# kwea123/nsff_pl

Hardware: AMD Instinct MI355X
Metric: ray-samples/sec (coarse+fine, static+dynamic) (higher is better)
Workload: dtype f16x3 (fp32 operands split into 2 halfs, 3 f16 MFMAs per product, fp32 accumulate; same 1e-4 parity as f32); 1 GPU; C2 (BASELINE.json configs[1]): static+dynamic NSFF, 1024 rays/GPU x (64 coarse + 64 importance -> 192 fine pts), train-mode fwd, fw/bw flow warp t+-1, perturb=1 noise_std=1, 8x256 MLPs, N_tau=48, all 47 outputs on device.  `value` is render_rays' throughput with autograd DISABLED (the train-mode FLAGS, inference launches: nothing kept for a backward pass); what a trainer's forward costs is aux.tra; rays_per_gpu=1024, N_samples=64, N_importance=64, parallelism=single GPU, field_launch=persistent (one workgroup per CU)

## Files before the change

include/nsff_render.h:

```cpp
#ifndef NSFF_RENDER_H
#define NSFF_RENDER_H

#include <stddef.h>
#include <stdint.h>

#ifdef __cplusplus
extern "C" {
#endif

#define NSFF_OK               0
#define NSFF_ERR_INVALID     -1
#define NSFF_ERR_NULL        -2
#define NSFF_ERR_ALIGN       -3
#define NSFF_ERR_HIP         -4

#define NSFF_ABI_VERSION      32
#define NSFF_RAW_STRIDE      16
#define NSFF_MAX_FREQS       24
#define NSFF_MAX_LAYERS       8


typedef struct NsffModelDesc {
    int32_t D;
    int32_t W;
// ... 287 lines not shown
    float* static_sigmas; float* transient_sigmas;
    float* static_alphas; float* transient_alphas;
    float* static_weights; float* transient_weights; float* weights;
    float* xyzs_fw_bw;   float* xyzs_bw_fw;
    float* disoccs_fw;   float* disoccs_bw;
    float* depth;  float* rgb;  float* transient_alpha;  float* transient_rgb;
    float* static_only_rgb;  float* static_only_depth;
    float* xyz_exp;  float* flow_fw_exp;  float* flow_bw_exp;  float* xyz_fw_exp;  float* xyz_bw_exp;
    float* rgb_fw;   float* rgb_bw;
    float* disocc_fw;  float* disocc_bw;
    NsffFrustumArgs vis;
} NsffCompositeArgs;

int nsff_composite(const NsffCompositeArgs* args, void* stream);

int nsff_frustum_visibility(const NsffFrustumArgs* vis, const float* xyz, int64_t n_points, float* vis_count,
                            void* stream);

typedef struct NsffSplatArgs {
    int32_t H, W, n_planes;
    float   K4[4];
    float   P[12];
    float   scale;
    const float* xyz;
    const float* flow;
    const float* rgb;
    const float* alpha;
    float*       accum;
    void*        work;
    int64_t      work_bytes;
// ... 112 lines not shown
```

nsff_pl_amd/_lib.py:

```python
import ctypes as C
import os

import torch

_HERE = os.path.dirname(os.path.abspath(__file__))
LIB_PATH = os.environ.get("NSFF_LIB") or os.path.join(_HERE, "libnsff_hip.so")

RAW_STRIDE = 16
ABI_VERSION = 32
MAX_FREQS = 24

_ERR = {-1: "NSFF_ERR_INVALID (bad shape/flag/unsupported architecture)",
        -2: "NSFF_ERR_NULL (required pointer missing)",
        -3: "NSFF_ERR_ALIGN (pointer not 16-byte aligned)",
        -4: "NSFF_ERR_HIP"}

_fp = C.c_void_p


class ModelDesc(C.Structure):
    _fields_ = [("D", C.c_int32), ("W", C.c_int32), ("skip", C.c_int32),
                ("in_xyz", C.c_int32), ("in_dir", C.c_int32), ("in_a", C.c_int32),
                ("in_t", C.c_int32), ("use_viewdir", C.c_int32),
                ("has_transient", C.c_int32), ("has_flow", C.c_int32),
# ... 161 lines not shown
    "nsff_param_count": (C.c_int, [C.POINTER(ModelDesc)]),
    "nsff_pack_weights": (C.c_int, [C.POINTER(ModelDesc), C.c_int, C.POINTER(_fp), _fp, _fp]),
    "nsff_pack_weights_ex": (C.c_int, [C.POINTER(ModelDesc), C.c_int, C.POINTER(_fp), _fp, C.c_int32, _fp]),
    "nsff_fold_heads": (C.c_int, [C.POINTER(ModelDesc), C.c_int, C.POINTER(_fp), _fp, _fp]),
    "nsff_posenc": (C.c_int, [_fp, C.c_int64, C.POINTER(C.c_float), C.c_int, _fp, _fp]),
    "nsff_time_rows": (C.c_int, [_fp, C.c_int64, C.c_int32, _fp, C.c_int64, C.c_int64, _fp, _fp, _fp]),
    "nsff_time_rows_backward": (C.c_int, [_fp, _fp, _fp, _fp, C.c_int64, C.c_int64, C.c_int64, C.c_int32, _fp, _fp]),
    "nsff_field_query": (C.c_int, [C.POINTER(ModelDesc), _fp, C.POINTER(FieldArgs), _fp]),
    "nsff_coarse_samples": (C.c_int, [_fp, C.c_int64, _fp, C.c_int32, C.c_float, _fp, _fp, _fp, _fp]),
    "nsff_fine_samples": (C.c_int, [_fp, C.c_int64, _fp, _fp, C.c_int32, C.c_int32, _fp, _fp, _fp, _fp,
                                    C.c_int32, _fp, _fp, _fp, _fp, _fp]),
    "nsff_sample_pdf": (C.c_int, [_fp, _fp, C.c_int64, C.c_int32, _fp, C.c_int32, C.c_int32,
                                  C.c_float, _fp, _fp]),
    "nsff_warp_points": (C.c_int, [_fp, _fp, _fp, C.c_int64, C.c_float, _fp, _fp, _fp]),
    "nsff_composite": (C.c_int, [C.POINTER(CompositeArgs), _fp]),
    "nsff_frustum_visibility": (C.c_int, [C.POINTER(FrustumArgs), _fp, C.c_int64, _fp, _fp]),
    "nsff_frame_rays": (C.c_int, [C.POINTER(C.c_float), C.POINTER(C.c_float), C.c_int32, C.c_int32, C.c_float,
                                  C.c_float, C.c_int64, C.c_int64, _fp, _fp]),
    "nsff_bwd_packed_bytes": (C.c_int, [C.POINTER(ModelDesc), C.POINTER(C.c_size_t)]),
    "nsff_pack_weights_bwd": (C.c_int, [C.POINTER(ModelDesc), C.POINTER(_fp), _fp, _fp]),
    "nsff_field_backward": (C.c_int, [C.POINTER(ModelDesc), _fp, C.POINTER(FieldBwdArgs), _fp]),
    "nsff_field_input_backward": (C.c_int, [_fp, C.c_int32, C.c_int32, _fp, C.c_int64, C.c_int32, C.POINTER(C.c_float), C.c_int32,
                                            C.c_int32, _fp, _fp, _fp]),
    "nsff_train_dims": (C.c_int, [C.POINTER(ModelDesc), C.POINTER(C.c_int32), C.POINTER(C.c_int32), C.POINTER(C.c_int32)]),
    "nsff_weight_grad_scratch": (C.c_int64, [C.POINTER(WgradJob), C.c_int32, C.c_int64, C.c_int32]),
    "nsff_weight_grad": (C.c_int, [C.POINTER(WgradJob), C.c_int32, C.c_int64, C.c_int32, _fp, _fp, _fp, _fp, _fp]),
    "nsff_weight_grad_accumulate": (C.c_int, [C.POINTER(WgradJob), C.c_int32, C.c_int64, C.c_int32, _fp, _fp, C.c_int64,
                                              _fp, _fp, _fp]),
    "nsff_weight_grad_accumulate_aux": (C.c_int, [C.POINTER(WgradJob), C.c_int32, C.c_int64, C.c_int32, _fp, _fp, C.c_int64,
                                                  _fp, _fp, _fp, _fp]),
# ... 17 lines not shown
    "nsff_nerfw_loss_work_bytes": (C.c_size_t, [C.c_longlong]),
    "nsff_nerfw_loss_ex": (C.c_int, [C.POINTER(LossArgs), C.c_int, _fp, C.c_size_t, _fp]),
    "nsff_last_loss_path": (C.c_int, []),
    "nsff_splat_planes": (C.c_int, [C.POINTER(SplatArgs), _fp]),
    "nsff_splat_work_bytes": (C.c_int64, [C.c_int32, C.c_int32, C.c_int32]),
    "nsff_mpi_composite": (C.c_int, [C.POINTER(MpiArgs), _fp]),
    "nsff_ssim_scratch_bytes": (C.c_int64, [C.c_int32, C.c_int32, C.c_int32]),
    "nsff_ssim": (C.c_int, [C.POINTER(SsimArgs), _fp]),
    "nsff_cdf": (C.c_int, [_fp, C.c_int64, C.c_int64, _fp, _fp]),
    "nsff_ray_draw": (C.c_int, [C.POINTER(RayDrawArgs), _fp]),
    "nsff_prof_enable": (C.c_int, [C.c_int]),
    "nsff_prof_collect": (C.c_int, [C.POINTER(C.c_int64), C.POINTER(C.c_double), C.POINTER(C.c_double), C.POINTER(C.c_double)]),
    "nsff_prof_collect_clock": (C.c_int, [C.POINTER(C.c_int64)] + [C.POINTER(C.c_double)] * 5),
}
EXPORTED_SYMBOLS = tuple(_SIGNATURES)

_lib = None


def load():
    global _lib
    if _lib is None:
        if not os.path.exists(LIB_PATH):
            raise RuntimeError(
                f"{LIB_PATH} is missing: build it with `python -c 'import __graft_entry__ as g; g.build()'` "
                "(or `make -C nsff_pl_amd/csrc`).  There is no CPU fallback for the render path.")
        lib = C.CDLL(LIB_PATH)
        for name, (res, args) in _SIGNATURES.items():
            fn = getattr(lib, name)
            fn.restype, fn.argtypes = res, args
        if lib.nsff_abi_version() != ABI_VERSION:
            raise RuntimeError("libnsff_hip.so ABI version mismatch")
        _lib = lib
    return _lib


def _check(rc, what):
    if rc != 0:
        msg = _ERR.get(rc, f"error {rc}")
        if rc == -4:
            msg += ": " + load().nsff_last_hip_error().decode()
        raise RuntimeError(f"{what} failed: {msg}")

# ... 358 lines not shown

def frustum_args(w2c, ts, K4, n_cams, n_frames, H, W):
    assert w2c.is_cuda and w2c.dtype == torch.float32 and w2c.is_contiguous() and w2c.shape == (n_cams * n_frames, 12)
    assert ts.is_cuda and ts.dtype == torch.int64 and ts.is_contiguous() and ts.numel() >= 1
    a = FrustumArgs(w2c=w2c.data_ptr(), ts=ts.data_ptr(), n_cams=int(n_cams), n_frames=int(n_frames), H=int(H), W=int(W))
    a.K4[:] = [float(v) for v in K4]
    a._keep = (w2c, ts)
    return a


def frustum_visibility(vis, xyz, out):
    _check(load().nsff_frustum_visibility(C.byref(vis), _ptr(xyz), xyz.shape[0], _ptr(out), _stream()),
           "nsff_frustum_visibility")


def composite(vis=None, **kw):
    a = CompositeArgs()
    for k, v in kw.items():
        if k in _COMPOSITE_PTRS_IN or k in _COMPOSITE_PTRS_OUT:
            setattr(a, k, _ptr(v))
        else:
            setattr(a, k, v)
    if vis is not None:
        a.vis = vis
    _check(load().nsff_composite(C.byref(a), _stream()), "nsff_composite")


def frame_rays(K4, c2w12, H, W, near, shift_near, first, count, rays):
    k = (C.c_float * 4)(*[float(v) for v in K4])
    m = (C.c_float * 12)(*[float(v) for v in c2w12])
    _check(load().nsff_frame_rays(k, m, int(H), int(W), float(near), float(shift_near), int(first), int(count),
                                  _ptr(rays), _stream()), "nsff_frame_rays")


BWD_PACK = 100


def bwd_packed_bytes(desc):
    n = C.c_size_t(0)
    _check(load().nsff_bwd_packed_bytes(C.byref(desc), C.byref(n)), "nsff_bwd_packed_bytes")
# ... 324 lines not shown
```

nsff_pl_amd/csrc/rays.hip:

```cpp
#include <hip/hip_runtime.h>
#include <cstdlib>
#include "nsff_common.h"

namespace {

constexpr int WAVES_PER_BLOCK = 4;
constexpr int RS = NSFF_RAW_STRIDE;

__device__ __forceinline__ float wave_sum(float v) {
#pragma unroll
    for (int off = 32; off > 0; off >>= 1) v += __shfl_xor(v, off);
    return v;
}

__device__ __forceinline__ float wave_scan_mul(float v, int lane) {
#pragma unroll
    for (int off = 1; off < 64; off <<= 1) {
        const float u = __shfl_up(v, off);
        if (lane >= off) v *= u;
    }
    return v;
}
__device__ __forceinline__ float wave_scan_add(float v, int lane) {
#pragma unroll
// ... 60 lines not shown
            if (out_b) out_b[k] = s;
        }
    }
    __syncthreads();
}

struct FineArgs {
    const float* rays; long long n_rays; const float* z_lin; const float* zs_coarse;
    int S, n_imp;
    const float* w_static; const float* w_transient;
    const float* u_static; const float* u_transient; int u_per_ray;
    float* samples_static; float* samples_transient;
    float* zs_fine; float* xyz_fine;
};

__global__ __launch_bounds__(64 * WAVES_PER_BLOCK) void fine_samples_kernel(const FineArgs a) {
    extern __shared__ __attribute__((aligned(16))) float smem[];
    const int lane = threadIdx.x & 63, wave = threadIdx.x >> 6, tid = threadIdx.x;
    constexpr int T = 64 * WAVES_PER_BLOCK;
    const long long ray = blockIdx.x;
    const int S = a.S, n_imp = a.n_imp;
    const int k_sets = a.w_transient ? 2 : 1;
    const int Sf = S + k_sets * n_imp;
    float* cdf = smem + wave * S;
    float* bins = smem + WAVES_PER_BLOCK * S;
    float* merged = bins + ((S + 3) & ~3);
    for (int j = tid; j < S - 1; j += T) bins[j] = 0.5f * (a.z_lin[j] + a.z_lin[j + 1]);
    for (int j = tid; j < S; j += T) merged[j] = a.zs_coarse[ray * S + j];
    __syncthreads();
    {
        const bool mine = wave < k_sets;
        const int set = mine ? wave : 0;
        const float* w = (set == 0 ? a.w_static : a.w_transient) + ray * S + 1;
        const float* ub = set == 0 ? a.u_static : a.u_transient;
        const float* u = a.u_per_ray ? ub + ray * n_imp : ub;
        float* keep = set == 0 ? a.samples_static : a.samples_transient;
        sample_pdf_ray(w, bins, S - 2, 1e-5f, u, n_imp, cdf, merged + S + set * n_imp,
                       keep ? keep + ray * n_imp : nullptr, lane, mine);
    }
    const float* r = a.rays + ray * 6;
    const float o0 = r[0], o1 = r[1], o2 = r[2], d0 = r[3], d1 = r[4], d2 = r[5];
    for (int i = tid; i < Sf; i += T) {
        const float v = merged[i];
        int rank = 0;
        int j = 0;
        for (; j + 4 <= Sf; j += 4) {
            const float4 o = *reinterpret_cast<const float4*>(merged + j);
            rank += (o.x < v || (o.x == v && j < i)) ? 1 : 0;
            rank += (o.y < v || (o.y == v && j + 1 < i)) ? 1 : 0;
            rank += (o.z < v || (o.z == v && j + 2 < i)) ? 1 : 0;
            rank += (o.w < v || (o.w == v && j + 3 < i)) ? 1 : 0;
        }
        for (; j < Sf; ++j) {
            const float o = merged[j];
            rank += (o < v || (o == v && j < i)) ? 1 : 0;
        }
        const long long dst = ray * Sf + rank;
        a.zs_fine[dst] = v;
        a.xyz_fine[dst * 3 + 0] = o0 + d0 * v;
        a.xyz_fine[dst * 3 + 1] = o1 + d1 * v;
        a.xyz_fine[dst * 3 + 2] = o2 + d2 * v;
    }
}

struct PdfArgs {
    const float* bins; const float* weights; long long n_rays; int M;
    const float* u; int n_imp; int u_per_ray; float eps; float* samples;
};

__global__ __launch_bounds__(64 * WAVES_PER_BLOCK) void sample_pdf_kernel(const PdfArgs a) {
    extern __shared__ __attribute__((aligned(16))) float smem[];
    const int lane = threadIdx.x & 63, wave = threadIdx.x >> 6;
    const long long ray_raw = (long long)blockIdx.x * WAVES_PER_BLOCK + wave;
    const bool active = ray_raw < a.n_rays;
    const long long ray = active ? ray_raw : a.n_rays - 1;
    float* cdf = smem + wave * (a.M + 1);
    const float* u = a.u_per_ray ? a.u + ray * a.n_imp : a.u;
// ... 66 lines not shown
        const float cam2 = fmaf(m[10], rz, fmaf(m[9], ry, m[8] * rx)) + m[11];
        if (!(cam2 < 0.f)) continue;
        const float c1 = -cam1, c2 = -cam2;
        const float u = fmaf(cx, c2, fx * cam0) / c2, w = fmaf(cy, c2, fy * c1) / c2;
        if (u >= 0.f && u < (float)v.W && w >= 0.f && w < (float)v.H) count += 1.f;
    }
    return count;
}

__global__ __launch_bounds__(256) void frustum_visibility_kernel(const NsffFrustumArgs v, const float* __restrict__ xyz,
                                                                 long long n_points, float* __restrict__ out) {
    const long long p = (long long)blockIdx.x * 256 + threadIdx.x;
    if (p < n_points) out[p] = frustum_count(v, xyz[3 * p], xyz[3 * p + 1], xyz[3 * p + 2]);
}

__global__ __launch_bounds__(64 * WAVES_PER_BLOCK) void composite_kernel(const NsffCompositeArgs a) {
    const int lane = threadIdx.x & 63;
    const long long ray = (long long)blockIdx.x * WAVES_PER_BLOCK + (threadIdx.x >> 6);
    if (ray >= a.n_rays) return;
    const int S = a.n_samples;
    const bool tr = a.has_transient != 0;
    const bool flows = tr && a.flow_mode >= 1;
    const bool warps = tr && a.flow_mode >= 2;

    float cT = 1.f, cTs = 1.f, cTfw = 1.f, cTbw = 1.f;
    float s_depth = 0.f, s_rgb[3] = {0, 0, 0}, s_talpha = 0.f, s_trgb[3] = {0, 0, 0};
    float s_sorgb[3] = {0, 0, 0}, s_sodepth = 0.f;
    float s_xyz[3] = {0, 0, 0}, s_ffw[3] = {0, 0, 0}, s_fbw[3] = {0, 0, 0};
    float s_rgbfw[3] = {0, 0, 0}, s_rgbbw[3] = {0, 0, 0}, s_occfw = 0.f, s_occbw = 0.f;

    for (int base = 0; base < S; base += 64) {
        const int i = base + lane;
        const bool on = i < S;
        const long long idx = ray * S + (on ? i : S - 1);
// ... 36 lines not shown
            if (a.has_rgb && a.static_rgbs) {
                a.static_rgbs[idx * 3 + 0] = rgb_s[0]; a.static_rgbs[idx * 3 + 1] = rgb_s[1];
                a.static_rgbs[idx * 3 + 2] = rgb_s[2];
            }
            if (tr) {
                if (a.transient_sigmas) a.transient_sigmas[idx] = sig_t;
                if (a.has_rgb && a.transient_rgbs) {
                    a.transient_rgbs[idx * 3 + 0] = rgb_t[0]; a.transient_rgbs[idx * 3 + 1] = rgb_t[1];
                    a.transient_rgbs[idx * 3 + 2] = rgb_t[2];
                }
                if (a.static_alphas) a.static_alphas[idx] = al_s;
                if (a.transient_alphas) a.transient_alphas[idx] = al_t;
                if (a.static_weights) a.static_weights[idx] = w_s;
                if (a.transient_weights) a.transient_weights[idx] = w_t;
                if (a.weights) a.weights[idx] = w;
            } else {
                if (a.static_weights) a.static_weights[idx] = w;
                if (a.weights) a.weights[idx] = w;
            }
        }
        if (!a.has_rgb) continue;

        if (on) {
            s_depth += w * z;
            if (tr) {
#pragma unroll
                for (int c = 0; c < 3; ++c) { s_rgb[c] += w_s * rgb_s[c]; s_trgb[c] += w_t * rgb_t[c]; }
                s_talpha += w_t;
            } else {
#pragma unroll
                for (int c = 0; c < 3; ++c) s_rgb[c] += w * rgb_s[c];
            }
        }
// ... 105 lines not shown
            if (a.flow_bw_exp) a.flow_bw_exp[ray * 3 + c] = s_fbw[c];
            if (a.xyz_fw_exp) a.xyz_fw_exp[ray * 3 + c] = s_xyz[c] + s_ffw[c];
            if (a.xyz_bw_exp) a.xyz_bw_exp[ray * 3 + c] = s_xyz[c] + s_fbw[c];
        }
    }
    if (warps) {
        for (int c = 0; c < 3; ++c) {
            if (a.rgb_fw) a.rgb_fw[ray * 3 + c] = s_rgbfw[c];
            if (a.rgb_bw) a.rgb_bw[ray * 3 + c] = s_rgbbw[c];
        }
        if (a.disocc_fw) a.disocc_fw[ray] = 1.f - fabsf(s_occfw);
        if (a.disocc_bw) a.disocc_bw[ray] = 1.f - fabsf(s_occbw);
    }
}

template <int NCH>
__global__ __launch_bounds__(64 * NCH) void composite_kernel_chunks(const NsffCompositeArgs a) {
    __shared__ float tot[NCH][4];
    __shared__ float part[NCH][32];
    const int lane = threadIdx.x & 63, c = threadIdx.x >> 6;
    const long long ray = blockIdx.x;
    const int S = a.n_samples;
    const bool tr = a.has_transient != 0;
    const bool flows = tr && a.flow_mode >= 1;
    const bool warps = tr && a.flow_mode >= 2;

    const int i = 64 * c + lane;
    const bool on = i < S;
    const long long idx = ray * S + (on ? i : S - 1);
    const float z = a.zs[idx];
    const bool last = i >= S - 1;
    const float dz = last ? 0.f : a.zs[idx + 1] - z;
    const float d_s = last ? 100.f : dz;
    const float d_t = last ? 1e-3f : dz;
    const float* rec = a.raw + idx * RS;

    float sig_s = rec[3];
    if (a.noise_static) sig_s += a.noise_static[idx] * a.noise_std;
    sig_s = softplus(sig_s);
    const float al_s = 1.f - expf(-d_s * sig_s);
    float rgb_s[3] = {0, 0, 0};
    if (a.has_rgb) { rgb_s[0] = rec[0]; rgb_s[1] = rec[1]; rgb_s[2] = rec[2]; }

    float sig_t = 0.f, al_t = 0.f, alpha = al_s;
    float rgb_t[3] = {0, 0, 0};
    if (tr) {
        sig_t = rec[7];
        if (a.visibility && a.visibility[idx] == 0.f) sig_t = -10.f;
        if (a.vis.w2c && frustum_count(a.vis, a.xyz[idx * 3], a.xyz[idx * 3 + 1], a.xyz[idx * 3 + 2]) == 0.f) sig_t = -10.f;
        if (a.noise_transient) sig_t += a.noise_transient[idx] * a.noise_std;
        sig_t = softplus(sig_t);
        al_t = 1.f - expf(-d_t * sig_t);
        alpha = 1.f - (1.f - al_s) * (1.f - al_t);
        if (a.has_rgb) { rgb_t[0] = rec[4]; rgb_t[1] = rec[5]; rgb_t[2] = rec[6]; }
    }
    const float inc = wave_scan_mul(on ? 1.f - alpha : 1.f, lane);
    float incs = 1.f, incw[2] = {1.f, 1.f}, al_tw[2] = {0.f, 0.f};
    if (a.has_rgb && tr) incs = wave_scan_mul(on ? 1.f - al_s : 1.f, lane);
    if (a.has_rgb && warps) {
#pragma unroll
        for (int dir = 0; dir < 2; ++dir) {
            const float* recw = (dir == 0 ? a.raw_fw : a.raw_bw) + idx * RS;
            const float* nz = dir == 0 ? a.noise_fw : a.noise_bw;
            float sg = recw[7];
            if (nz) sg += nz[idx] * a.noise_std;
            al_tw[dir] = 1.f - expf(-d_t * softplus(sg));
            const float al_w = 1.f - (1.f - al_s) * (1.f - al_tw[dir]);
            incw[dir] = wave_scan_mul(on ? 1.f - al_w : 1.f, lane);
        }
    }
    if (lane == 63) { tot[c][0] = inc; tot[c][1] = incs; tot[c][2] = incw[0]; tot[c][3] = incw[1]; }
    __syncthreads();
    float cT = 1.f, cTs = 1.f, cTw[2] = {1.f, 1.f};
    for (int cc = 0; cc < c; ++cc) { cT *= tot[cc][0]; cTs *= tot[cc][1]; cTw[0] *= tot[cc][2]; cTw[1] *= tot[cc][3]; }

    float exc = __shfl_up(inc, 1);
    if (lane == 0) exc = 1.f;
    const float T = cT * exc;
    const float w = alpha * T, w_s = al_s * T, w_t = al_t * T;
    if (on) {
        if (a.static_sigmas) a.static_sigmas[idx] = sig_s;
        if (a.has_rgb && a.static_rgbs) {
            a.static_rgbs[idx * 3 + 0] = rgb_s[0]; a.static_rgbs[idx * 3 + 1] = rgb_s[1];
            a.static_rgbs[idx * 3 + 2] = rgb_s[2];
        }
        if (tr) {
            if (a.transient_sigmas) a.transient_sigmas[idx] = sig_t;
            if (a.has_rgb && a.transient_rgbs) {
                a.transient_rgbs[idx * 3 + 0] = rgb_t[0]; a.transient_rgbs[idx * 3 + 1] = rgb_t[1];
                a.transient_rgbs[idx * 3 + 2] = rgb_t[2];
            }
            if (a.static_alphas) a.static_alphas[idx] = al_s;
            if (a.transient_alphas) a.transient_alphas[idx] = al_t;
            if (a.static_weights) a.static_weights[idx] = w_s;
            if (a.transient_weights) a.transient_weights[idx] = w_t;
            if (a.weights) a.weights[idx] = w;
        } else {
            if (a.static_weights) a.static_weights[idx] = w;
            if (a.weights) a.weights[idx] = w;
        }
    }
    if (!a.has_rgb) return;

    enum { P_DEPTH, P_RGB, P_TRGB = P_RGB + 3, P_TALPHA = P_TRGB + 3, P_SORGB, P_SODEPTH = P_SORGB + 3, P_XYZ, P_FFW = P_XYZ + 3,
           P_FBW = P_FFW + 3, P_RGBFW = P_FBW + 3, P_RGBBW = P_RGBFW + 3, P_OCCFW = P_RGBBW + 3, P_OCCBW, P_N };
    static_assert(P_N <= 32, "part[] columns");
    float p[P_N];
#pragma unroll
    for (int k = 0; k < P_N; ++k) p[k] = 0.f;
    if (on) {
        p[P_DEPTH] = w * z;
        if (tr) {
#pragma unroll
            for (int k = 0; k < 3; ++k) { p[P_RGB + k] = w_s * rgb_s[k]; p[P_TRGB + k] = w_t * rgb_t[k]; }
            p[P_TALPHA] = w_t;
        } else {
#pragma unroll
// ... 3 lines not shown
    if (tr) {
        float excs = __shfl_up(incs, 1);
        if (lane == 0) excs = 1.f;
        const float wso = al_s * (cTs * excs);
        if (on) {
#pragma unroll
            for (int k = 0; k < 3; ++k) p[P_SORGB + k] = wso * rgb_s[k];
            p[P_SODEPTH] = wso * z;
        }
    }
    if (flows) {
        const bool far = z > a.z_far;
        float ffw[3], fbw[3], x[3];
#pragma unroll
        for (int k = 0; k < 3; ++k) {
            ffw[k] = far ? 0.f : rec[8 + k];
            fbw[k] = far ? 0.f : rec[11 + k];
            x[k] = a.xyz[idx * 3 + k];
        }
        if (on) {
#pragma unroll
            for (int k = 0; k < 3; ++k) {
                if (a.flows_fw) a.flows_fw[idx * 3 + k] = ffw[k];
                if (a.flows_bw) a.flows_bw[idx * 3 + k] = fbw[k];
                p[P_XYZ + k] = w * x[k]; p[P_FFW + k] = w * ffw[k]; p[P_FBW + k] = w * fbw[k];
            }
        }
        if (warps) {
#pragma unroll
            for (int dir = 0; dir < 2; ++dir) {
                const float* recw = (dir == 0 ? a.raw_fw : a.raw_bw) + idx * RS;
                float excw = __shfl_up(incw[dir], 1);
                if (lane == 0) excw = 1.f;
                const float Tw = cTw[dir] * excw;
                const float ws_w = al_s * Tw, wt_w = al_tw[dir] * Tw;
                if (on) {
#pragma unroll
                    for (int k = 0; k < 3; ++k) p[(dir == 0 ? P_RGBFW : P_RGBBW) + k] = ws_w * rgb_s[k] + wt_w * recw[4 + k];
                    const float* xw = (dir == 0 ? a.xyz_fw : a.xyz_bw) + idx * 3;
                    float* cyc = dir == 0 ? a.xyzs_fw_bw : a.xyzs_bw_fw;
                    const int head = dir == 0 ? 11 : 8;
                    if (cyc) {
#pragma unroll
                        for (int k = 0; k < 3; ++k) cyc[idx * 3 + k] = xw[k] + (far ? 0.f : recw[head + k]);
                    }
                    const float occ = wt_w - w_t;
                    if (dir == 0) { p[P_OCCFW] = occ; if (a.disoccs_fw) a.disoccs_fw[idx] = 1.f - fabsf(occ); }
                    else          { p[P_OCCBW] = occ; if (a.disoccs_bw) a.disoccs_bw[idx] = 1.f - fabsf(occ); }
                }
            }
        }
    }
    const int n_used = warps ? (int)P_N : (flows ? (int)P_RGBFW : (tr ? (int)P_XYZ : (int)P_TRGB));
#pragma unroll
    for (int k = 0; k < P_N; ++k) {
        if (k < n_used) {
            const float v = wave_sum(p[k]);
            if (lane == 0) part[c][k] = v;
        }
    }
    __syncthreads();
    if (threadIdx.x != 0) return;
    float s[P_N];
// ... 239 lines not shown

int nsff_composite(const NsffCompositeArgs* args, void* stream) {
    if (!args) return NSFF_ERR_NULL;
    const NsffCompositeArgs& a = *args;
    if (a.n_rays < 0 || a.n_samples < 1 || a.flow_mode < 0 || a.flow_mode > 2) return NSFF_ERR_INVALID;
    if (a.n_rays == 0) return NSFF_OK;
    if (!a.raw || !a.zs) return NSFF_ERR_NULL;
    if (a.flow_mode && (!a.has_transient || !a.has_rgb)) return NSFF_ERR_INVALID;
    if (a.flow_mode >= 1 && !a.xyz) return NSFF_ERR_NULL;
    if (a.flow_mode == 2 && (!a.raw_fw || !a.raw_bw || !a.xyz_fw || !a.xyz_bw)) return NSFF_ERR_NULL;
    if (a.vis.w2c && (!a.vis.ts || !a.xyz)) return NSFF_ERR_NULL;
    if (a.vis.w2c && (a.vis.n_cams < 1 || a.vis.n_frames < 1)) return NSFF_ERR_INVALID;
    const int nch = (a.n_samples + 63) / 64;
    if (nch >= 2 && nch <= 4 && a.n_rays <= 0x7fffffffLL && getenv("NSFF_SERIAL_COMPOSITE") == nullptr) {
        const dim3 grid((unsigned)a.n_rays);
        if (nch == 2) hipLaunchKernelGGL(composite_kernel_chunks<2>, grid, dim3(128), 0, (hipStream_t)stream, a);
        else if (nch == 3) hipLaunchKernelGGL(composite_kernel_chunks<3>, grid, dim3(192), 0, (hipStream_t)stream, a);
        else hipLaunchKernelGGL(composite_kernel_chunks<4>, grid, dim3(256), 0, (hipStream_t)stream, a);
        return nsff_launch_status();
    }
    const unsigned blocks = (unsigned)((a.n_rays + WAVES_PER_BLOCK - 1) / WAVES_PER_BLOCK);
    hipLaunchKernelGGL(composite_kernel, dim3(blocks), dim3(64 * WAVES_PER_BLOCK), 0,
                       (hipStream_t)stream, a);
    return nsff_launch_status();
}

int nsff_frustum_visibility(const NsffFrustumArgs* vis, const float* xyz, int64_t n_points, float* vis_count,
                            void* stream) {
    if (!vis || !vis->w2c || !vis->ts) return NSFF_ERR_NULL;
    if (n_points < 0 || vis->n_cams < 1 || vis->n_frames < 1) return NSFF_ERR_INVALID;
    if (n_points == 0) return NSFF_OK;
    if (!xyz || !vis_count) return NSFF_ERR_NULL;
    const long long blocks = (n_points + 255) / 256;
    if (blocks > 0x7fffffffLL) return NSFF_ERR_INVALID;
    hipLaunchKernelGGL(frustum_visibility_kernel, dim3((unsigned)blocks), dim3(256), 0, (hipStream_t)stream, *vis, xyz,
                       (long long)n_points, vis_count);
    return nsff_launch_status();
}
// ... 3 lines not shown
```

nsff_pl_amd/rendering.py:

```python
import os

import torch

from . import _lib
from . import autograd
from . import config
from . import range_check
from . import field_grad
from . import ray_geometry

Z_FAR = 0.95

def _new(ref, *shape):
    return torch.empty(*shape, device=ref.device, dtype=torch.float32)


def sample_pdf(bins, weights, N_importance, det=False, eps=1e-5):
    _lib.require_gpu_tensor(bins, "sample_pdf bins")
    bins = bins.contiguous().float()
    weights = weights.contiguous().float()
    n_rays = weights.shape[0]
    if det:
        u = torch.linspace(0, 1, N_importance, device=bins.device)
    else:
# ... 122 lines not shown
            ctx.neighbour_rows = (rows[1], rows[-1])
        return rows[0]
    t_embedded = override if override is not None else ctx.embeddings['t'](ts)
    t_embedded = t_embedded.detach().contiguous().float()
    plan = [p for p in plan if t_embedded.shape == (n_rays, p[2].in_channels_t)]
    if plan:
        if any(w == 'fw' for _, w, _, _ in plan):
            ctx.neighbour_rows = _neighbour_time_rows(ctx.embeddings, ts, ctx.max_t)
        src = {0: t_embedded, 1: ctx.neighbour_rows[0] if ctx.neighbour_rows else None, -1: ctx.neighbour_rows[1] if ctx.neighbour_rows else None}
        for (typ, which, _, _), out in zip(plan, _lib.time_bias([(mod, src[d]) for _, _, mod, d in plan])):
            ctx.tbias[(typ, which)] = out
    return t_embedded


def _inference(results, ctx, model, xyz, zs, output_transient, output_transient_flow,
               t_embedded, a_embedded):
    typ = model.typ
    n_rays, S = zs.shape
    test_time = ctx.test_time
    results[f'zs_{typ}'] = zs
    results[f'xyzs_{typ}'] = xyz
    P = n_rays * S
    sigma_only = typ == 'coarse' and test_time
    want_flow = bool(output_transient_flow) and output_transient and not sigma_only
    warps = want_flow and not test_time
    disocc = warps and 'disocc' in output_transient_flow
    if want_flow and not hasattr(model, "transient_flow_fw"):
        raise AttributeError(f"{typ} model has no flow heads")

    raw = _new(zs, P, _lib.RAW_STRIDE)
    side = dict(dir_emb=ctx.dir_embedded if model.use_viewdir and not sigma_only else None,
# ... 107 lines not shown
            args['transient_rgb'] = out(f'transient_rgb_{typ}', n_rays, 3)
            args['static_only_rgb'] = out(f'_static_rgb_{typ}', n_rays, 3)
            args['static_only_depth'] = out(f'_static_depth_{typ}', n_rays)
            if want_flow:
                args['flow_mode'] = 2 if warps else 1
                args['xyz_exp'] = out('xyz_fine', n_rays, 3)
                args['flow_fw_exp'] = out('transient_flow_fw', n_rays, 3)
                args['xyz_fw_exp'] = out('xyz_fw', n_rays, 3)
                args['flow_bw_exp'] = out('transient_flow_bw', n_rays, 3)
                args['xyz_bw_exp'] = out('xyz_bw', n_rays, 3)
                if disocc:
                    args['disocc_fw'] = out('disocc_fw', n_rays, 1)
                    args['disoccs_fw'] = out('disoccs_fw', n_rays, S, 1)
                    args['disocc_bw'] = out('disocc_bw', n_rays, 1)
                    args['disoccs_bw'] = out('disoccs_bw', n_rays, S, 1)
    if n_rays:
        _lib.composite(**args)


def render_rays(models,
                embeddings,
                rays,
                ts,
                max_t,
                N_samples=64,
                perturb=0,
                noise_std=0,
                N_importance=0,
                chunk=1024 * 32,
                test_time=False,
                **kwargs):
    _lib.require_gpu_tensor(rays, "rays")
# ... 30 lines not shown
        z_lin = _unit_linspace(N_samples, rays.device)
        zs = _new(rays, n_rays, N_samples)
        xyz_coarse = _new(rays, n_rays, N_samples, 3)
        ctx.draws = _Draws(rays.device, n_rays, N_samples, N_importance, perturb, noise_std, test_time, models, kwargs,
                           coarse=(rays, z_lin, zs, xyz_coarse))
        perturb_rand = ctx.draws.take("rand", n_rays, N_samples) if perturb > 0 else None
        if n_rays and not ctx.draws.coarse_done:
            _lib.coarse_samples(rays, z_lin, perturb, perturb_rand, zs, xyz_coarse)

        t_embedded = None
        if N_importance > 0:
            model = models['coarse']
            output_transient = bool(kwargs.get('output_transient', True) and model.encode_transient)
            t_embedded = _time_codes(ctx, models, kwargs, N_samples, N_importance, output_transient,
                                     kwargs.get('output_transient_flow', []))
            _inference(results, ctx, model, xyz_coarse, zs, output_transient, [], t_embedded, None)

            det = perturb == 0
            if det:
                u_s = _unit_linspace(N_importance, rays.device)
                u_t = u_s
            else:
                u_s = ctx.draws.take("rand", n_rays, N_importance)
                u_t = ctx.draws.take("rand", n_rays, N_importance) if output_transient else None
            S_fine = N_samples + (2 if output_transient else 1) * N_importance
            zs_static = _new(rays, n_rays, N_importance) if test_time else None
            zs_transient = _new(rays, n_rays, N_importance) if (test_time and output_transient) else None
            zs_fine = _new(rays, n_rays, S_fine)
            xyz_fine = _new(rays, n_rays, S_fine, 3)
            if n_rays:
                _lib.fine_samples(rays, z_lin, zs, N_importance,
                                  results['static_weights_coarse'],
                                  results['transient_weights_coarse'] if output_transient else None,
                                  u_s, u_t if output_transient else None, 0 if det else 1,
                                  zs_static, zs_transient, zs_fine, xyz_fine)
            if test_time:
                results['static_zs_fine'] = zs_static
                if output_transient:
                    results['transient_zs_fine'] = zs_transient
            if fine_points is not None:
                zs_fine, xyz_fine = fine_points(rays, zs_fine, xyz_fine)
                if tuple(zs_fine.shape) != (n_rays, S_fine) or tuple(xyz_fine.shape) != (n_rays, S_fine, 3):
                    raise ValueError(f"fine_points: expected shapes {(n_rays, S_fine)} / {(n_rays, S_fine, 3)}")
            zs, xyz = zs_fine, xyz_fine
        else:
# ... 24 lines not shown
```

Measured before the change: 66.14 million ray-samples/s.

## Fuse coarse composite with fine sampling and prefetch records in chunked composite

Adds a coarse_to_fine kernel. In it, one wave composites each coarse ray and writes the static and transient weights into LDS, and the remaining waves then build the PDF and draw fine samples from those LDS weights. This removes a kernel launch and the global round trip of the coarse weights between the two stages. It also adds a prefetching variant of the chunked composite kernel for flow_mode 2. That variant loads the raw, warp and xyz records up front with nontemporal vector loads and writes its outputs with nontemporal stores, aiming to overlap memory latency. The costs are that three waves sit idle during the fused composite phase, the fused path is limited to 64 coarse samples, and the kernel needs extra LDS.

```diff
diff --git a/include/nsff_render.h b/include/nsff_render.h
--- a/include/nsff_render.h
+++ b/include/nsff_render.h
@@ -325,6 +325,10 @@
 
 int nsff_composite(const NsffCompositeArgs* args, void* stream);
 
+int nsff_coarse_to_fine(const NsffCompositeArgs* args, const float* rays, const float* z_lin, int32_t n_importance,
+                        const float* u_static, const float* u_transient, int32_t u_per_ray,
+                        float* samples_static, float* samples_transient, float* zs_fine, float* xyz_fine, void* stream);
+
 int nsff_frustum_visibility(const NsffFrustumArgs* vis, const float* xyz, int64_t n_points, float* vis_count,
                             void* stream);
 
diff --git a/nsff_pl_amd/_lib.py b/nsff_pl_amd/_lib.py
--- a/nsff_pl_amd/_lib.py
+++ b/nsff_pl_amd/_lib.py
@@ -199,6 +199,7 @@
                                   C.c_float, _fp, _fp]),
     "nsff_warp_points": (C.c_int, [_fp, _fp, _fp, C.c_int64, C.c_float, _fp, _fp, _fp]),
     "nsff_composite": (C.c_int, [C.POINTER(CompositeArgs), _fp]),
+    "nsff_coarse_to_fine": (C.c_int, [C.POINTER(CompositeArgs), _fp, _fp, C.c_int32, _fp, _fp, C.c_int32, _fp, _fp, _fp, _fp, _fp]),
     "nsff_frustum_visibility": (C.c_int, [C.POINTER(FrustumArgs), _fp, C.c_int64, _fp, _fp]),
     "nsff_frame_rays": (C.c_int, [C.POINTER(C.c_float), C.POINTER(C.c_float), C.c_int32, C.c_int32, C.c_float,
                                   C.c_float, C.c_int64, C.c_int64, _fp, _fp]),
@@ -246,6 +247,7 @@
     "nsff_prof_collect_clock": (C.c_int, [C.POINTER(C.c_int64)] + [C.POINTER(C.c_double)] * 5),
 }
 EXPORTED_SYMBOLS = tuple(_SIGNATURES)
+_ADDED_SYMBOLS = ("nsff_coarse_to_fine",)
 
 _lib = None
 
@@ -259,6 +261,8 @@
                 "(or `make -C nsff_pl_amd/csrc`).  There is no CPU fallback for the render path.")
         lib = C.CDLL(LIB_PATH)
         for name, (res, args) in _SIGNATURES.items():
+            if name in _ADDED_SYMBOLS and not hasattr(lib, name):
+                continue
             fn = getattr(lib, name)
             fn.restype, fn.argtypes = res, args
         if lib.nsff_abi_version() != ABI_VERSION:
@@ -647,7 +651,7 @@
            "nsff_frustum_visibility")
 
 
-def composite(vis=None, **kw):
+def _composite_args(vis, kw):
     a = CompositeArgs()
     for k, v in kw.items():
         if k in _COMPOSITE_PTRS_IN or k in _COMPOSITE_PTRS_OUT:
@@ -656,7 +660,24 @@
             setattr(a, k, v)
     if vis is not None:
         a.vis = vis
-    _check(load().nsff_composite(C.byref(a), _stream()), "nsff_composite")
+    return a
+
+
+def composite(vis=None, **kw):
+    _check(load().nsff_composite(C.byref(_composite_args(vis, kw)), _stream()), "nsff_composite")
+
+
+def coarse_to_fine(composite_kw, rays, z_lin, n_importance, u_static, u_transient, u_per_ray, samples_static, samples_transient,
+                   zs_fine, xyz_fine):
+    lib = load()
+    if not hasattr(lib, "nsff_coarse_to_fine"):
+        raise RuntimeError(f"{LIB_PATH} has no nsff_coarse_to_fine: it was built from older sources; rebuild it "
+                           "(`make -C nsff_pl_amd/csrc`) or set NSFF_NO_FUSED_STAGES=1 to render with the separate launches")
+    kw = dict(composite_kw)
+    a = _composite_args(kw.pop("vis", None), kw)
+    _check(lib.nsff_coarse_to_fine(C.byref(a), _ptr(rays), _ptr(z_lin), int(n_importance), _ptr(u_static), _ptr(u_transient),
+                                   int(u_per_ray), _ptr(samples_static), _ptr(samples_transient), _ptr(zs_fine), _ptr(xyz_fine),
+                                   _stream()), "nsff_coarse_to_fine")
 
 
 def frame_rays(K4, c2w12, H, W, near, shift_near, first, count, rays):
diff --git a/nsff_pl_amd/csrc/rays.hip b/nsff_pl_amd/csrc/rays.hip
--- a/nsff_pl_amd/csrc/rays.hip
+++ b/nsff_pl_amd/csrc/rays.hip
@@ -6,6 +6,7 @@
 
 constexpr int WAVES_PER_BLOCK = 4;
 constexpr int RS = NSFF_RAW_STRIDE;
+typedef float f4v __attribute__((ext_vector_type(4)));
 
 __device__ __forceinline__ float wave_sum(float v) {
 #pragma unroll
@@ -98,24 +99,25 @@
     float* zs_fine; float* xyz_fine;
 };
 
-__global__ __launch_bounds__(64 * WAVES_PER_BLOCK) void fine_samples_kernel(const FineArgs a) {
-    extern __shared__ __attribute__((aligned(16))) float smem[];
+__device__ __forceinline__ void fine_samples_ray(const FineArgs& a, const long long ray, float* smem, const float* w_static,
+                                                 const float* w_transient, const int stage_tid, const int stage_T) {
     const int lane = threadIdx.x & 63, wave = threadIdx.x >> 6, tid = threadIdx.x;
     constexpr int T = 64 * WAVES_PER_BLOCK;
-    const long long ray = blockIdx.x;
     const int S = a.S, n_imp = a.n_imp;
-    const int k_sets = a.w_transient ? 2 : 1;
+    const int k_sets = w_transient ? 2 : 1;
     const int Sf = S + k_sets * n_imp;
     float* cdf = smem + wave * S;
     float* bins = smem + WAVES_PER_BLOCK * S;
     float* merged = bins + ((S + 3) & ~3);
-    for (int j = tid; j < S - 1; j += T) bins[j] = 0.5f * (a.z_lin[j] + a.z_lin[j + 1]);
-    for (int j = tid; j < S; j += T) merged[j] = a.zs_coarse[ray * S + j];
+    if (stage_tid >= 0) {
+        for (int j = stage_tid; j < S - 1; j += stage_T) bins[j] = 0.5f * (a.z_lin[j] + a.z_lin[j + 1]);
+        for (int j = stage_tid; j < S; j += stage_T) merged[j] = a.zs_coarse[ray * S + j];
+    }
     __syncthreads();
     {
         const bool mine = wave < k_sets;
         const int set = mine ? wave : 0;
-        const float* w = (set == 0 ? a.w_static : a.w_transient) + ray * S + 1;
+        const float* w = (set == 0 ? w_static : w_transient) + 1;
         const float* ub = set == 0 ? a.u_static : a.u_transient;
         const float* u = a.u_per_ray ? ub + ray * n_imp : ub;
         float* keep = set == 0 ? a.samples_static : a.samples_transient;
@@ -145,6 +147,13 @@
         a.xyz_fine[dst * 3 + 1] = o1 + d1 * v;
         a.xyz_fine[dst * 3 + 2] = o2 + d2 * v;
     }
+}
+
+__global__ __launch_bounds__(64 * WAVES_PER_BLOCK) void fine_samples_kernel(const FineArgs a) {
+    extern __shared__ __attribute__((aligned(16))) float smem[];
+    const long long ray = blockIdx.x;
+    fine_samples_ray(a, ray, smem, a.w_static + ray * a.S, a.w_transient ? a.w_transient + ray * a.S : nullptr,
+                     threadIdx.x, 64 * WAVES_PER_BLOCK);
 }
 
 struct PdfArgs {
@@ -241,10 +250,8 @@
     if (p < n_points) out[p] = frustum_count(v, xyz[3 * p], xyz[3 * p + 1], xyz[3 * p + 2]);
 }
 
-__global__ __launch_bounds__(64 * WAVES_PER_BLOCK) void composite_kernel(const NsffCompositeArgs a) {
-    const int lane = threadIdx.x & 63;
-    const long long ray = (long long)blockIdx.x * WAVES_PER_BLOCK + (threadIdx.x >> 6);
-    if (ray >= a.n_rays) return;
+__device__ __forceinline__ void composite_ray(const NsffCompositeArgs& a, const long long ray, const int lane,
+                                              float* lds_ws, float* lds_wt) {
     const int S = a.n_samples;
     const bool tr = a.has_transient != 0;
     const bool flows = tr && a.flow_mode >= 1;
@@ -311,9 +318,12 @@
                 if (a.static_weights) a.static_weights[idx] = w_s;
                 if (a.transient_weights) a.transient_weights[idx] = w_t;
                 if (a.weights) a.weights[idx] = w;
+                if (lds_ws) lds_ws[i] = w_s;
+                if (lds_wt) lds_wt[i] = w_t;
             } else {
                 if (a.static_weights) a.static_weights[idx] = w;
                 if (a.weights) a.weights[idx] = w;
+                if (lds_ws) lds_ws[i] = w;
             }
         }
         if (!a.has_rgb) continue;
@@ -449,56 +459,103 @@
     }
 }
 
-template <int NCH>
+__global__ __launch_bounds__(64 * WAVES_PER_BLOCK) void composite_kernel(const NsffCompositeArgs a) {
+    const long long ray = (long long)blockIdx.x * WAVES_PER_BLOCK + (threadIdx.x >> 6);
+    if (ray >= a.n_rays) return;
+    composite_ray(a, ray, threadIdx.x & 63, nullptr, nullptr);
+}
+
+__global__ __launch_bounds__(64 * WAVES_PER_BLOCK) void coarse_to_fine_kernel(const NsffCompositeArgs c, const FineArgs a) {
+    extern __shared__ __attribute__((aligned(16))) float smem[];
+    const long long ray = blockIdx.x;
+    const int S = a.S;
+    float* ws = smem + WAVES_PER_BLOCK * S + ((S + 3) & ~3) + ((S + 2 * a.n_imp + 3) & ~3);
+    float* wt = ws + S;
+    if (threadIdx.x < 64) composite_ray(c, ray, threadIdx.x, ws, c.has_transient ? wt : nullptr);
+    fine_samples_ray(a, ray, smem, ws, c.has_transient ? wt : nullptr, (int)threadIdx.x - 64, 64 * (WAVES_PER_BLOCK - 1));
+}
+
+template <int NCH, bool PRE>
 __global__ __launch_bounds__(64 * NCH) void composite_kernel_chunks(const NsffCompositeArgs a) {
     __shared__ float tot[NCH][4];
     __shared__ float part[NCH][32];
     const int lane = threadIdx.x & 63, c = threadIdx.x >> 6;
     const long long ray = blockIdx.x;
     const int S = a.n_samples;
-    const bool tr = a.has_transient != 0;
-    const bool flows = tr && a.flow_mode >= 1;
-    const bool warps = tr && a.flow_mode >= 2;
+    const bool tr = PRE || a.has_transient != 0;
+    const bool flows = PRE || (tr && a.flow_mode >= 1);
+    const bool warps = PRE || (tr && a.flow_mode >= 2);
+    const bool has_rgb = PRE || a.has_rgb != 0;
 
     const int i = 64 * c + lane;
     const bool on = i < S;
     const long long idx = ray * S + (on ? i : S - 1);
-    const float z = a.zs[idx];
     const bool last = i >= S - 1;
-    const float dz = last ? 0.f : a.zs[idx + 1] - z;
+    const float* rec = a.raw + idx * RS;
+    f4v q[4], qw[2][4];
+    float pz = 0.f, pzn = 0.f, pn_s = 0.f, pn_t = 0.f, pn_w[2] = {0.f, 0.f}, pvis = 1.f, px[3] = {0.f, 0.f, 0.f};
+    float pxw[2][3] = {{0.f, 0.f, 0.f}, {0.f, 0.f, 0.f}};
+    if constexpr (PRE) {
+        auto opt = [&](const float* ptr) { return (ptr ? ptr : a.zs)[idx]; };
+        pz = a.zs[idx];
+        pzn = a.zs[last ? idx : idx + 1];
+#pragma unroll
+        for (int j = 0; j < 4; ++j) q[j] = __builtin_nontemporal_load(reinterpret_cast<const f4v*>(rec) + j);
+#pragma unroll
+        for (int dir = 0; dir < 2; ++dir) {
+            const f4v* recw = reinterpret_cast<const f4v*>((dir == 0 ? a.raw_fw : a.raw_bw) + idx * RS);
+#pragma unroll
+            for (int j = 0; j < 4; ++j) qw[dir][j] = __builtin_nontemporal_load(recw + j);
+            const float* xw = (dir == 0 ? a.xyz_fw : a.xyz_bw) + idx * 3;
+#pragma unroll
+            for (int k = 0; k < 3; ++k) pxw[dir][k] = xw[k];
+        }
+#pragma unroll
+        for (int k = 0; k < 3; ++k) px[k] = a.xyz[idx * 3 + k];
+        pn_s = opt(a.noise_static); pn_t = opt(a.noise_transient); pn_w[0] = opt(a.noise_fw); pn_w[1] = opt(a.noise_bw);
+        pvis = opt(a.visibility);
+    }
+    auto R = [&](int k) -> float { if constexpr (PRE) return q[k >> 2][k & 3]; else return rec[k]; };
+    auto RW = [&](int dir, int k) -> float {
+        if constexpr (PRE) return qw[dir][k >> 2][k & 3]; else return ((dir == 0 ? a.raw_fw : a.raw_bw) + idx * RS)[k];
+    };
+    auto X = [&](int k) -> float { if constexpr (PRE) return px[k]; else return a.xyz[idx * 3 + k]; };
+    auto put = [&](float* dst, float v) { if constexpr (PRE) __builtin_nontemporal_store(v, dst); else *dst = v; };
+
+    float z, dz;
+    if constexpr (PRE) { z = pz; dz = last ? 0.f : pzn - z; }
+    else { z = a.zs[idx]; dz = last ? 0.f : a.zs[idx + 1] - z; }
     const float d_s = last ? 100.f : dz;
     const float d_t = last ? 1e-3f : dz;
-    const float* rec = a.raw + idx * RS;
-
-    float sig_s = rec[3];
-    if (a.noise_static) sig_s += a.noise_static[idx] * a.noise_std;
+
+    float sig_s = R(3);
+    if (a.noise_static) sig_s += (PRE ? pn_s : a.noise_static[idx]) * a.noise_std;
     sig_s = softplus(sig_s);
     const float al_s = 1.f - expf(-d_s * sig_s);
     float rgb_s[3] = {0, 0, 0};
-    if (a.has_rgb) { rgb_s[0] = rec[0]; rgb_s[1] = rec[1]; rgb_s[2] = rec[2]; }
+    if (has_rgb) { rgb_s[0] = R(0); rgb_s[1] = R(1); rgb_s[2] = R(2); }
 
     float sig_t = 0.f, al_t = 0.f, alpha = al_s;
     float rgb_t[3] = {0, 0, 0};
     if (tr) {
-        sig_t = rec[7];
-        if (a.visibility && a.visibility[idx] == 0.f) sig_t = -10.f;
-        if (a.vis.w2c && frustum_count(a.vis, a.xyz[idx * 3], a.xyz[idx * 3 + 1], a.xyz[idx * 3 + 2]) == 0.f) sig_t = -10.f;
-        if (a.noise_transient) sig_t += a.noise_transient[idx] * a.noise_std;
+        sig_t = R(7);
+        if (a.visibility && (PRE ? pvis : a.visibility[idx]) == 0.f) sig_t = -10.f;
+        if (a.vis.w2c && frustum_count(a.vis, X(0), X(1), X(2)) == 0.f) sig_t = -10.f;
+        if (a.noise_transient) sig_t += (PRE ? pn_t : a.noise_transient[idx]) * a.noise_std;
         sig_t = softplus(sig_t);
         al_t = 1.f - expf(-d_t * sig_t);
         alpha = 1.f - (1.f - al_s) * (1.f - al_t);
-        if (a.has_rgb) { rgb_t[0] = rec[4]; rgb_t[1] = rec[5]; rgb_t[2] = rec[6]; }
+        if (has_rgb) { rgb_t[0] = R(4); rgb_t[1] = R(5); rgb_t[2] = R(6); }
     }
     const float inc = wave_scan_mul(on ? 1.f - alpha : 1.f, lane);
     float incs = 1.f, incw[2] = {1.f, 1.f}, al_tw[2] = {0.f, 0.f};
-    if (a.has_rgb && tr) incs = wave_scan_mul(on ? 1.f - al_s : 1.f, lane);
-    if (a.has_rgb && warps) {
+    if (has_rgb && tr) incs = wave_scan_mul(on ? 1.f - al_s : 1.f, lane);
+    if (has_rgb && warps) {
 #pragma unroll
         for (int dir = 0; dir < 2; ++dir) {
-            const float* recw = (dir == 0 ? a.raw_fw : a.raw_bw) + idx * RS;
             const float* nz = dir == 0 ? a.noise_fw : a.noise_bw;
-            float sg = recw[7];
-            if (nz) sg += nz[idx] * a.noise_std;
+            float sg = RW(dir, 7);
+            if (nz) sg += (PRE ? pn_w[dir] : nz[idx]) * a.noise_std;
             al_tw[dir] = 1.f - expf(-d_t * softplus(sg));
             const float al_w = 1.f - (1.f - al_s) * (1.f - al_tw[dir]);
             incw[dir] = wave_scan_mul(on ? 1.f - al_w : 1.f, lane);
@@ -514,28 +571,28 @@
     const float T = cT * exc;
     const float w = alpha * T, w_s = al_s * T, w_t = al_t * T;
     if (on) {
-        if (a.static_sigmas) a.static_sigmas[idx] = sig_s;
-        if (a.has_rgb && a.static_rgbs) {
-            a.static_rgbs[idx * 3 + 0] = rgb_s[0]; a.static_rgbs[idx * 3 + 1] = rgb_s[1];
-            a.static_rgbs[idx * 3 + 2] = rgb_s[2];
+        if (a.static_sigmas) put(a.static_sigmas + idx, sig_s);
+        if (has_rgb && a.static_rgbs) {
+            put(a.static_rgbs + idx * 3 + 0, rgb_s[0]); put(a.static_rgbs + idx * 3 + 1, rgb_s[1]);
+            put(a.static_rgbs + idx * 3 + 2, rgb_s[2]);
         }
         if (tr) {
-            if (a.transient_sigmas) a.transient_sigmas[idx] = sig_t;
-            if (a.has_rgb && a.transient_rgbs) {
-                a.transient_rgbs[idx * 3 + 0] = rgb_t[0]; a.transient_rgbs[idx * 3 + 1] = rgb_t[1];
-                a.transient_rgbs[idx * 3 + 2] = rgb_t[2];
-            }
-            if (a.static_alphas) a.static_alphas[idx] = al_s;
-            if (a.transient_alphas) a.transient_alphas[idx] = al_t;
-            if (a.static_weights) a.static_weights[idx] = w_s;
-            if (a.transient_weights) a.transient_weights[idx] = w_t;
-            if (a.weights) a.weights[idx] = w;
+            if (a.transient_sigmas) put(a.transient_sigmas + idx, sig_t);
+            if (has_rgb && a.transient_rgbs) {
+                put(a.transient_rgbs + idx * 3 + 0, rgb_t[0]); put(a.transient_rgbs + idx * 3 + 1, rgb_t[1]);
+                put(a.transient_rgbs + idx * 3 + 2, rgb_t[2]);
+            }
+            if (a.static_alphas) put(a.static_alphas + idx, al_s);
+            if (a.transient_alphas) put(a.transient_alphas + idx, al_t);
+            if (a.static_weights) put(a.static_weights + idx, w_s);
+            if (a.transient_weights) put(a.transient_weights + idx, w_t);
+            if (a.weights) put(a.weights + idx, w);
         } else {
-            if (a.static_weights) a.static_weights[idx] = w;
-            if (a.weights) a.weights[idx] = w;
-        }
-    }
-    if (!a.has_rgb) return;
+            if (a.static_weights) put(a.static_weights + idx, w);
+            if (a.weights) put(a.weights + idx, w);
+        }
+    }
+    if (!has_rgb) return;
 
     enum { P_DEPTH, P_RGB, P_TRGB = P_RGB + 3, P_TALPHA = P_TRGB + 3, P_SORGB, P_SODEPTH = P_SORGB + 3, P_XYZ, P_FFW = P_XYZ + 3,
            P_FBW = P_FFW + 3, P_RGBFW = P_FBW + 3, P_RGBBW = P_RGBFW + 3, P_OCCFW = P_RGBBW + 3, P_OCCBW, P_N };
@@ -569,39 +626,38 @@
         float ffw[3], fbw[3], x[3];
 #pragma unroll
         for (int k = 0; k < 3; ++k) {
-            ffw[k] = far ? 0.f : rec[8 + k];
-            fbw[k] = far ? 0.f : rec[11 + k];
-            x[k] = a.xyz[idx * 3 + k];
+            ffw[k] = far ? 0.f : R(8 + k);
+            fbw[k] = far ? 0.f : R(11 + k);
+            x[k] = X(k);
         }
         if (on) {
 #pragma unroll
             for (int k = 0; k < 3; ++k) {
-                if (a.flows_fw) a.flows_fw[idx * 3 + k] = ffw[k];
-                if (a.flows_bw) a.flows_bw[idx * 3 + k] = fbw[k];
+                if (a.flows_fw) put(a.flows_fw + idx * 3 + k, ffw[k]);
+                if (a.flows_bw) put(a.flows_bw + idx * 3 + k, fbw[k]);
                 p[P_XYZ + k] = w * x[k]; p[P_FFW + k] = w * ffw[k]; p[P_FBW + k] = w * fbw[k];
             }
         }
         if (warps) {
 #pragma unroll
             for (int dir = 0; dir < 2; ++dir) {
-                const float* recw = (dir == 0 ? a.raw_fw : a.raw_bw) + idx * RS;
                 float excw = __shfl_up(incw[dir], 1);
                 if (lane == 0) excw = 1.f;
                 const float Tw = cTw[dir] * excw;
                 const float ws_w = al_s * Tw, wt_w = al_tw[dir] * Tw;
                 if (on) {
 #pragma unroll
-                    for (int k = 0; k < 3; ++k) p[(dir == 0 ? P_RGBFW : P_RGBBW) + k] = ws_w * rgb_s[k] + wt_w * recw[4 + k];
+                    for (int k = 0; k < 3; ++k) p[(dir == 0 ? P_RGBFW : P_RGBBW) + k] = ws_w * rgb_s[k] + wt_w * RW(dir, 4 + k);
                     const float* xw = (dir == 0 ? a.xyz_fw : a.xyz_bw) + idx * 3;
                     float* cyc = dir == 0 ? a.xyzs_fw_bw : a.xyzs_bw_fw;
-                    const int head = dir == 0 ? 11 : 8;
                     if (cyc) {
 #pragma unroll
-                        for (int k = 0; k < 3; ++k) cyc[idx * 3 + k] = xw[k] + (far ? 0.f : recw[head + k]);
+                        for (int k = 0; k < 3; ++k)
+                            put(cyc + idx * 3 + k, (PRE ? pxw[dir][k] : xw[k]) + (far ? 0.f : RW(dir, (dir == 0 ? 11 : 8) + k)));
                     }
                     const float occ = wt_w - w_t;
-                    if (dir == 0) { p[P_OCCFW] = occ; if (a.disoccs_fw) a.disoccs_fw[idx] = 1.f - fabsf(occ); }
-                    else          { p[P_OCCBW] = occ; if (a.disoccs_bw) a.disoccs_bw[idx] = 1.f - fabsf(occ); }
+                    if (dir == 0) { p[P_OCCFW] = occ; if (a.disoccs_fw) put(a.disoccs_fw + idx, 1.f - fabsf(occ)); }
+                    else          { p[P_OCCBW] = occ; if (a.disoccs_bw) put(a.disoccs_bw + idx, 1.f - fabsf(occ)); }
                 }
             }
         }
@@ -871,14 +927,38 @@
     const int nch = (a.n_samples + 63) / 64;
     if (nch >= 2 && nch <= 4 && a.n_rays <= 0x7fffffffLL && getenv("NSFF_SERIAL_COMPOSITE") == nullptr) {
         const dim3 grid((unsigned)a.n_rays);
-        if (nch == 2) hipLaunchKernelGGL(composite_kernel_chunks<2>, grid, dim3(128), 0, (hipStream_t)stream, a);
-        else if (nch == 3) hipLaunchKernelGGL(composite_kernel_chunks<3>, grid, dim3(192), 0, (hipStream_t)stream, a);
-        else hipLaunchKernelGGL(composite_kernel_chunks<4>, grid, dim3(256), 0, (hipStream_t)stream, a);
+        const bool pre = a.flow_mode == 2 && (((uintptr_t)a.raw | (uintptr_t)a.raw_fw | (uintptr_t)a.raw_bw) & 15) == 0 &&
+                         getenv("NSFF_NO_COMPOSITE_PREFETCH") == nullptr;
+        void (*kernel)(const NsffCompositeArgs) =
+            nch == 2 ? (pre ? composite_kernel_chunks<2, true> : composite_kernel_chunks<2, false>)
+          : nch == 3 ? (pre ? composite_kernel_chunks<3, true> : composite_kernel_chunks<3, false>)
+                     : (pre ? composite_kernel_chunks<4, true> : composite_kernel_chunks<4, false>);
+        hipLaunchKernelGGL(kernel, grid, dim3(64 * nch), 0, (hipStream_t)stream, a);
         return nsff_launch_status();
     }
     const unsigned blocks = (unsigned)((a.n_rays + WAVES_PER_BLOCK - 1) / WAVES_PER_BLOCK);
     hipLaunchKernelGGL(composite_kernel, dim3(blocks), dim3(64 * WAVES_PER_BLOCK), 0,
                        (hipStream_t)stream, a);
+    return nsff_launch_status();
+}
+
+int nsff_coarse_to_fine(const NsffCompositeArgs* args, const float* rays, const float* z_lin, int32_t n_importance,
+                        const float* u_static, const float* u_transient, int32_t u_per_ray,
+                        float* samples_static, float* samples_transient, float* zs_fine, float* xyz_fine, void* stream) {
+    if (!args) return NSFF_ERR_NULL;
+    const NsffCompositeArgs& c = *args;
+    if (c.n_rays < 0 || c.n_samples != 64 || c.flow_mode != 0 || n_importance < 1) return NSFF_ERR_INVALID;
+    if (c.n_rays == 0) return NSFF_OK;
+    if (!c.raw || !c.zs || !rays || !z_lin || !u_static || !zs_fine || !xyz_fine) return NSFF_ERR_NULL;
+    if (c.has_transient && !u_transient) return NSFF_ERR_NULL;
+    if (c.vis.w2c && (!c.vis.ts || !c.xyz)) return NSFF_ERR_NULL;
+    if (c.vis.w2c && (c.vis.n_cams < 1 || c.vis.n_frames < 1)) return NSFF_ERR_INVALID;
+    const int S = c.n_samples;
+    FineArgs a{rays, (long long)c.n_rays, z_lin, c.zs, S, n_importance, nullptr, nullptr, u_static, u_transient, u_per_ray,
+               samples_static, samples_transient, zs_fine, xyz_fine};
+    const size_t lds = (size_t)(WAVES_PER_BLOCK * S + ((S + 3) & ~3) + ((S + 2 * n_importance + 3) & ~3) + 2 * S) * sizeof(float);
+    if (lds > 64 * 1024 || c.n_rays > 0x7fffffffLL) return NSFF_ERR_INVALID;
+    hipLaunchKernelGGL(coarse_to_fine_kernel, dim3((unsigned)c.n_rays), dim3(64 * WAVES_PER_BLOCK), lds, (hipStream_t)stream, c, a);
     return nsff_launch_status();
 }
 
diff --git a/nsff_pl_amd/rendering.py b/nsff_pl_amd/rendering.py
--- a/nsff_pl_amd/rendering.py
+++ b/nsff_pl_amd/rendering.py
@@ -160,7 +160,7 @@
 
 
 def _inference(results, ctx, model, xyz, zs, output_transient, output_transient_flow,
-               t_embedded, a_embedded):
+               t_embedded, a_embedded, defer_composite=False):
     typ = model.typ
     n_rays, S = zs.shape
     test_time = ctx.test_time
@@ -298,8 +298,11 @@
                     args['disoccs_fw'] = out('disoccs_fw', n_rays, S, 1)
                     args['disocc_bw'] = out('disocc_bw', n_rays, 1)
                     args['disoccs_bw'] = out('disoccs_bw', n_rays, S, 1)
+    if defer_composite:
+        return args
     if n_rays:
         _lib.composite(**args)
+    return None
 
 
 def render_rays(models,
@@ -360,7 +363,9 @@
             output_transient = bool(kwargs.get('output_transient', True) and model.encode_transient)
             t_embedded = _time_codes(ctx, models, kwargs, N_samples, N_importance, output_transient,
                                      kwargs.get('output_transient_flow', []))
-            _inference(results, ctx, model, xyz_coarse, zs, output_transient, [], t_embedded, None)
+            fused = (N_samples == 64 and fine_points is None and not os.environ.get('NSFF_NO_FUSED_STAGES'))
+            coarse_args = _inference(results, ctx, model, xyz_coarse, zs, output_transient, [], t_embedded, None,
+                                     defer_composite=fused)
 
             det = perturb == 0
             if det:
@@ -374,7 +379,10 @@
             zs_transient = _new(rays, n_rays, N_importance) if (test_time and output_transient) else None
             zs_fine = _new(rays, n_rays, S_fine)
             xyz_fine = _new(rays, n_rays, S_fine, 3)
-            if n_rays:
+            if n_rays and fused:
+                _lib.coarse_to_fine(coarse_args, rays, z_lin, N_importance, u_s, u_t if output_transient else None,
+                                    0 if det else 1, zs_static, zs_transient, zs_fine, xyz_fine)
+            elif n_rays:
                 _lib.fine_samples(rays, z_lin, zs, N_importance,
                                   results['static_weights_coarse'],
                                   results['transient_weights_coarse'] if output_transient else None,
```

Measured after the change: 66.40 million ray-samples/s (median of 6 runs). Within noise of the previous version (+0.4%).
